# aymenboudhina/Multimodal_VQVAE_compression_audio_tactile

Hardware: AMD Instinct MI355X
Metric: encode+VQ+decode token-frames/sec (1 frame = 13.33 ms of paired 24 kHz audio+tactile) (higher is better)
Workload: dtype f32

## Files before the change

### multimodal_vqvae_compression_audio_tactile_amd/csrc/conv1d_mfma.hpp

```cpp
#pragma once
#include <hip/hip_runtime.h>
#include <stdio.h>
#include <stdlib.h>
#include <type_traits>
#include "det_math.hpp"
#include "kernels_small.hpp"

namespace mvq {

struct ConvArgs;
inline bool conv_dma_rows_ok(const ConvArgs& a);

__device__ __attribute__((aligned(16))) static const float g_zero16[4] = {0.0f, 0.0f, 0.0f, 0.0f};

int prof_begin(const char* kernel_name, double flops, hipStream_t s);
void prof_end(int idx, hipStream_t s);
bool prof_enabled();

typedef float f32x16 __attribute__((ext_vector_type(16)));
typedef float f32x4 __attribute__((ext_vector_type(4)));

struct ConvArgs {
    const float* x;
    const float* wp;
// ... 212 lines not shown
            __builtin_amdgcn_sched_barrier(0);
            run_from<S + 1>(acc, av0, bv0, av1, bv1, a_addr, b_same, b_cross);
        }
    }
};

constexpr int cgcd(int a, int b) { return b == 0 ? a : cgcd(b, a % b); }

template <int KS, int STRIDE, int DIL, int CK, int MT, int NT, int WAVES_M, int WAVES_N, int UPS>
struct ConvCfg {
    static constexpr int BM = 32 * MT * WAVES_M;
    static constexpr int BN = 32 * NT * WAVES_N;
    static constexpr int KC = CK * KS;
    static constexpr int XT = (BN - 1) * STRIDE + (KS - 1) * DIL + 1;
    static constexpr bool XALIGNED = (KS == 1 && STRIDE == 1);
    static constexpr int XV = XALIGNED ? (XT + 3) / 4 : (XT + 3 + 3) / 4;
    static constexpr int XTP = XV * 4 + 4;
    static constexpr int W_FLOATS = KC * BM;
    static constexpr int X_FLOATS = CK * XTP;
    static constexpr int STAGE_FLOATS = 2 * (W_FLOATS + X_FLOATS);
    static constexpr int BNP = BN + 4;
    static constexpr int CT_FLOATS = BM * BNP;
    static constexpr int EH = ((UPS == 0 || 32 % (UPS ? UPS : 1) == 0) && MT % 2 == 0 && CT_FLOATS > STAGE_FLOATS) ? 2 : 1;
    static constexpr int CTH_FLOATS = CT_FLOATS / EH;
    static constexpr int QPR = BN / 4;
    static constexpr int CQ = cgcd(QPR, 64 * WAVES_M * WAVES_N);
    static constexpr int JN = QPR / CQ;
    static constexpr int RSTEP = (64 * WAVES_M * WAVES_N) / CQ;
    static constexpr bool REG_GEOM = (UPS == 0) && (32 % RSTEP == 0);
    static constexpr int TB_FLOATS = REG_GEOM ? 2 * BM : 0;
    static constexpr int EPI_FLOATS = CTH_FLOATS + TB_FLOATS;
    static constexpr int EPI_FLOATS_FUSE = CT_FLOATS + TB_FLOATS;
    static constexpr int LDS_FLOATS = STAGE_FLOATS > EPI_FLOATS ? STAGE_FLOATS : EPI_FLOATS;
    static constexpr bool FOUR_WAVES = WAVES_M * WAVES_N == 4;
    static constexpr bool RING_FITS = (size_t)3 * (KC * BM + CK * XV * 4) * 4 <= 64 * 1024;
    static constexpr int MIN_WPE = (FOUR_WAVES && LDS_FLOATS * 4 <= 53 * 1024 && !(WAVES_N == 4 && NT == 2) && RING_FITS && MT * NT <= 4) ? 3
                                                                                                                : (WAVES_M * WAVES_N) / 2;
    static constexpr int LDS_FLOATS_FUSE = STAGE_FLOATS > EPI_FLOATS_FUSE ? STAGE_FLOATS : EPI_FLOATS_FUSE;
    static constexpr int MIN_WPE_FUSE = (FOUR_WAVES && (LDS_FLOATS_FUSE + 5 * BM) * 4 * 3 <= 160 * 1024) ? 3 : (WAVES_M * WAVES_N) / 2;
    static constexpr int XV4 = XV * 4;
    static constexpr int DMA_STAGE_FLOATS = W_FLOATS + CK * XV4;
    static constexpr int DMA_NV = DMA_STAGE_FLOATS / 4;
    static constexpr int DMA_NU = (DMA_NV + 64 * WAVES_M * WAVES_N - 1) / (64 * WAVES_M * WAVES_N);
    static constexpr int LDS_FLOATS_DMA = 3 * DMA_STAGE_FLOATS > EPI_FLOATS ? 3 * DMA_STAGE_FLOATS : EPI_FLOATS;
    static constexpr int LDS_FLOATS_FUSE_DMA = 3 * DMA_STAGE_FLOATS > EPI_FLOATS_FUSE ? 3 * DMA_STAGE_FLOATS : EPI_FLOATS_FUSE;
    static constexpr int W_VEC = W_FLOATS / 4;
    static constexpr int NTHR = 64 * WAVES_M * WAVES_N;
    static constexpr int W_PER_THREAD = (W_VEC + NTHR - 1) / NTHR;
    static constexpr int XV_TOTAL = CK * XV;
    static constexpr int XV_PER_THREAD = (XV_TOTAL + NTHR - 1) / NTHR;
    static constexpr int XS_TOTAL = CK * XT;
    static constexpr int XS_PER_THREAD = (XS_TOTAL + NTHR - 1) / NTHR;
    static constexpr int XREGS = (4 * XV_PER_THREAD > XS_PER_THREAD) ? 4 * XV_PER_THREAD : XS_PER_THREAD;
    static_assert(WAVES_M * WAVES_N == 4 || WAVES_M * WAVES_N == 8, "block is 4 or 8 waves");
    static_assert(KC % 2 == 0, "chunk K must be even (32x32x2 MFMA)");
    static_assert(BM % 4 == 0, "float4 weight staging");
};

template <int KS, int STRIDE, int DIL, int CK, int MT, int NT, int WAVES_M, int WAVES_N, int UPS, bool VEC>
struct ConvTile {
    using C = ConvCfg<KS, STRIDE, DIL, CK, MT, NT, WAVES_M, WAVES_N, UPS>;
    const float* wp; const float* xb; const float* Al;
    float* Ws; float* Xs;
    int tid, Tin, Cin, Mpad, m0, t_in0, g_al;
    bool snake_in;

    __device__ __forceinline__ void load_chunk(int chunk, f32x4 (&wreg)[C::W_PER_THREAD], f32x4 (&xv)[C::XV_PER_THREAD], float (&xs)[C::XS_PER_THREAD]) const
    {
        const int ci0 = chunk * CK;
        const float* wsrc = wp + (size_t)ci0 * KS * Mpad + m0;
#pragma unroll
        for (int u = 0; u < C::W_PER_THREAD; ++u) {
            int v = tid + u * C::NTHR;
            if (C::W_VEC % C::NTHR != 0) v = v < C::W_VEC ? v : C::W_VEC - 1;
            const int row = v / (C::BM / 4);
            const int c4 = v - row * (C::BM / 4);
            wreg[u] = *reinterpret_cast<const f32x4*>(wsrc + (size_t)row * Mpad + c4 * 4);
        }
        if (VEC) {
#pragma unroll
            for (int u = 0; u < C::XV_PER_THREAD; ++u) {
                int e = tid + u * C::NTHR;
                if (C::XV_TOTAL % C::NTHR != 0) e = e < C::XV_TOTAL ? e : C::XV_TOTAL - 1;
                const int cl = e / C::XV;
                const int v = e - cl * C::XV;
                const int g = g_al + 4 * v;
                const bool ok = g >= 0 && g < Tin;
                const int gc = ok ? g : 0;
                xv[u] = *reinterpret_cast<const f32x4*>(xb + (size_t)(ci0 + cl) * Tin + gc);
            }
        } else {
#pragma unroll
            for (int u = 0; u < C::XS_PER_THREAD; ++u) {
                int e = tid + u * C::NTHR;
                if (C::XS_TOTAL % C::NTHR != 0) e = e < C::XS_TOTAL ? e : C::XS_TOTAL - 1;
                const int cl = e / C::XT;
                const int xi = e - cl * C::XT;
                const int g = t_in0 + xi;
                const bool ok = g >= 0 && g < Tin;
                const int gc = ok ? g : 0;
                xs[u] = xb[(size_t)(ci0 + cl) * Tin + gc];
            }
        }
    }

    __device__ __forceinline__ void store_chunk(int chunk, int buf, const f32x4 (&wreg)[C::W_PER_THREAD],
                                                const f32x4 (&xv)[C::XV_PER_THREAD],
                                                const float (&xs)[C::XS_PER_THREAD]) const
    {
        const int ci0 = chunk * CK;
        float* wdst = Ws + buf * C::W_FLOATS;
        float* xdst = Xs + buf * C::X_FLOATS;
#pragma unroll
        for (int u = 0; u < C::W_PER_THREAD; ++u) {
            const int v = tid + u * C::NTHR;
            if (C::W_VEC % C::NTHR == 0 || v < C::W_VEC) *reinterpret_cast<f32x4*>(wdst + v * 4) = wreg[u];
        }
        if (VEC) {
#pragma unroll
            for (int u = 0; u < C::XV_PER_THREAD; ++u) {
                const int e = tid + u * C::NTHR;
                const int ec = (C::XV_TOTAL % C::NTHR != 0 && e >= C::XV_TOTAL) ? C::XV_TOTAL - 1 : e;
                const int cl = ec / C::XV;
                const int v = ec - cl * C::XV;
                const int g = g_al + 4 * v;
                const bool ok = g >= 0 && g < Tin;
                f32x4 q = xv[u];
                if (!ok) q = f32x4{0.0f, 0.0f, 0.0f, 0.0f};
                if (snake_in) {
                    const float al = Al[ci0 + cl], inv = Al[Cin + ci0 + cl];
                    q.x = det_snake(q.x, al, inv); q.y = det_snake(q.y, al, inv);
                    q.z = det_snake(q.z, al, inv); q.w = det_snake(q.w, al, inv);
                }
                if (C::XV_TOTAL % C::NTHR == 0 || e < C::XV_TOTAL)
                    *reinterpret_cast<f32x4*>(xdst + cl * C::XTP + 4 * v) = q;
            }
        } else {
#pragma unroll
            for (int u = 0; u < C::XS_PER_THREAD; ++u) {
                const int e = tid + u * C::NTHR;
                const int ec = (C::XS_TOTAL % C::NTHR != 0 && e >= C::XS_TOTAL) ? C::XS_TOTAL - 1 : e;
                const int cl = ec / C::XT;
                const int xi = ec - cl * C::XT;
                const int g = t_in0 + xi;
                float q = (g >= 0 && g < Tin) ? xs[u] : 0.0f;
                if (snake_in) q = det_snake(q, Al[ci0 + cl], Al[Cin + ci0 + cl]);
                if (C::XS_TOTAL % C::NTHR == 0 || e < C::XS_TOTAL) xdst[cl * C::XTP + xi] = q;
            }
        }
    }
};

template <int KS, int STRIDE, int DIL, int CK, int MT, int NT, int WAVES_M, int WAVES_N, int UPS, bool VEC, bool FUSE>
__device__ __forceinline__ void conv1d_mfma_body(const ConvArgs& a)
{
    using C = ConvCfg<KS, STRIDE, DIL, CK, MT, NT, WAVES_M, WAVES_N, UPS>;
    extern __shared__ __attribute__((aligned(16))) float smem[];
    float* const Ws = smem;
    float* const Xs = smem + 2 * C::W_FLOATS;
    float* const Ep = smem + (FUSE ? (a.dma ? C::LDS_FLOATS_FUSE_DMA : C::LDS_FLOATS_FUSE) : (a.dma ? C::LDS_FLOATS_DMA : C::LDS_FLOATS));
    constexpr int EP_MID = 2;
    float* const Al = Ep + 3 * C::BM;

    const int tid = threadIdx.x;
    const int lane = tid & 63;
    const int wave = tid >> 6;
    const int wm = wave / WAVES_N;
    const int wn = wave % WAVES_N;
    const int l31 = lane & 31;
    const int h = lane >> 5;

    int bx = blockIdx.x, by = blockIdx.y;
    if (a.row_fast) {
        const int xcd = bx & 7, j = bx >> 3;
        by = j % a.row_fast;
        bx = (j / a.row_fast) * 8 + xcd;
        if (bx >= a.n_tiles * a.B) return;
    }
    const int b = bx / a.n_tiles;
    const int tile_n = bx - b * a.n_tiles;
    const int n0 = a.n_base + tile_n * C::BN;
    const int m0 = by * C::BM;
    const int t_in0 = n0 * STRIDE - a.pad;
    const int g_al = t_in0 & ~3;
    const int shift = VEC ? (t_in0 - g_al) : 0;
    const int Cin = a.Cin;
    const int n_chunks = Cin / CK;
    const bool snake_in = a.alpha_in != nullptr;

    if (snake_in) {
        for (int c = tid; c < Cin; c += C::NTHR) {
            const float al = a.alpha_in[c];
            Al[c] = al;
            Al[Cin + c] = 1.0f / (al + 1e-9f);
        }
    }
    for (int r = tid; r < C::BM; r += C::NTHR) {
        int m = m0 + r;
        m = m < a.Mrows ? m : a.Mrows - 1;
        const int ch = m / (UPS ? UPS : 1);
        const float* tabs[4] = {a.alpha_out, a.y2 ? a.alpha2 : nullptr, FUSE ? a.alpha_mid : (a.dsn_src ? a.dsn_alpha : nullptr), nullptr};
#pragma unroll
        for (int k = 0; k < 3; ++k) {
            Ep[k * C::BM + r] = tabs[k] ? 1.0f / (tabs[k][ch] + 1e-9f) : 1.0f;
        }
    }

    ConvTile<KS, STRIDE, DIL, CK, MT, NT, WAVES_M, WAVES_N, UPS, VEC> tile;
    tile.wp = a.wp; tile.xb = a.x + (size_t)b * Cin * a.Tin; tile.Al = Al; tile.Ws = Ws; tile.Xs = Xs;
    tile.tid = tid; tile.Tin = a.Tin; tile.Cin = Cin; tile.Mpad = a.Mpad; tile.m0 = m0; tile.t_in0 = t_in0;
    tile.g_al = g_al; tile.snake_in = snake_in;

    f32x16 acc[MT][NT];
#pragma unroll
    for (int i = 0; i < MT; ++i)
#pragma unroll
        for (int j = 0; j < NT; ++j)
#pragma unroll
            for (int r = 0; r < 16; ++r) acc[i][j][r] = 0.0f;

    f32x4 wreg[C::W_PER_THREAD];
    f32x4 xv[C::XV_PER_THREAD];
    float xs[C::XS_PER_THREAD];

    constexpr int D_SAME = DIL;
    constexpr int D_CROSS = C::XTP - (KS - 1) * DIL;
    const int a_base = h * C::BM + wm * (MT * 32) + l31;
    const int b_base = (wn * (NT * 32) + l31) * STRIDE + shift;
    const int b_same = b_base + h * D_SAME;
    const int b_cross = b_base + h * D_CROSS;

    constexpr int NS = C::KC / 2;
    auto mfma_chunk = [&](int buf) __attribute__((always_inline)) {
        const float* wsrc = Ws + buf * C::W_FLOATS + a_base;
        const float* xs_same = Xs + buf * C::X_FLOATS + b_same;
        const float* xs_cross = Xs + buf * C::X_FLOATS + b_cross;
        float av[2][MT], bv[2][NT];
        auto load_step = [&](int st, int pb) __attribute__((always_inline)) {
            const int k0 = 2 * st;
            const int off0 = (k0 / KS) * C::XTP + (k0 % KS) * DIL;
            const bool cross = ((k0 + 1) / KS) != (k0 / KS);
            const float* xsp = cross ? xs_cross : xs_same;
#pragma unroll
            for (int i = 0; i < MT; ++i) av[pb][i] = wsrc[k0 * C::BM + i * 32];
#pragma unroll
            for (int j = 0; j < NT; ++j) bv[pb][j] = xsp[off0 + j * 32 * STRIDE];
        };
        load_step(0, 0);
#pragma unroll
        for (int s = 0; s < NS; ++s) {
            const int pb = s & 1;
            if (s + 1 < NS) load_step(s + 1, (s + 1) & 1);
#pragma unroll
            for (int i = 0; i < MT; ++i)
#pragma unroll
                for (int j = 0; j < NT; ++j)
                    acc[i][j] = __builtin_amdgcn_mfma_f32_32x32x2f32(av[pb][i], bv[pb][j], acc[i][j], 0, 0, 0);
            __builtin_amdgcn_sched_group_barrier(0x100, MT + NT, 0);
            __builtin_amdgcn_sched_group_barrier(0x008, MT * NT, 0);
        }
    };

    constexpr bool DMA_FITS = FUSE ? ((size_t)C::LDS_FLOATS_FUSE_DMA + 3 * C::BM) * 4 * 2 <= 160 * 1024 : (size_t)C::LDS_FLOATS_DMA * 4 <= 64 * 1024;
    bool use_dma = false;
    if constexpr (VEC && DMA_FITS) use_dma = a.dma != 0;
    if (use_dma) {
      if constexpr (VEC && DMA_FITS) {
        constexpr int NU = C::DMA_NU;
        constexpr int XP = C::XV4;
        constexpr int D_CROSS_D = XP - (KS - 1) * DIL;
        const int bd_same = b_base + h * D_SAME;
        const int bd_cross = b_base + h * D_CROSS_D;
        const unsigned lds0 = (unsigned)(size_t)smem;
        const int wave_u = __builtin_amdgcn_readfirstlane(wave);
        using AL = AsmOperandLoop<KS, STRIDE, DIL, C::BM, XP, MT, NT, NS>;
        auto chunk_rt = [&](int stage, auto&& issue) __attribute__((always_inline)) {
            const unsigned sb = lds0 + (unsigned)(stage * C::DMA_STAGE_FLOATS * 4);
            const unsigned a_addr = sb + (unsigned)(a_base * 4);
            const unsigned b_s = sb + (unsigned)((C::W_FLOATS + bd_same) * 4), b_c = sb + (unsigned)((C::W_FLOATS + bd_cross) * 4);
            float av0[MT], bv0[NT], av1[MT], bv1[NT];
            AL::template load_step<0>(av0, bv0, a_addr, b_s, b_c);
            issue();
            AL::template run_from<0>(acc, av0, bv0, av1, bv1, a_addr, b_s, b_c);
        };
        constexpr int NW = WAVES_M * WAVES_N;
        constexpr int XPC = CK * C::XV;
        constexpr int WI_W = (C::W_VEC + 63) / 64, WI_X = (XPC + 63) / 64;
        constexpr int NU_W = (WI_W + NW - 1) / NW, NU_X = (WI_X + NW - 1) / NW;
        constexpr int NF_W = C::W_VEC / C::NTHR, NF_X = XPC / C::NTHR;
        static_assert(NU_W - NF_W <= 1 && NU_X - NF_X <= 1, "at most one masked instruction per kind");
        constexpr int NI_MIN = (WI_W + WI_X) / NW;
        constexpr bool UNI_OK = (size_t)3 * C::DMA_STAGE_FLOATS * 4 <= 65536 && NF_W <= 8 && NF_X <= 8;
        bool uni = false;
        if constexpr (UNI_OK) uni = !a.vp_seg && g_al >= 0 && g_al + 4 * C::XV <= a.Tin && (long long)CK * a.Tin < (1ll << 29);
        if (uni) {
          if constexpr (UNI_OK) {
            unsigned woff[NU_W], xoff[NU_X];
#pragma unroll
            for (int u = 0; u < NU_W; ++u) {
                int p = tid + u * C::NTHR;
                p = p < C::W_VEC ? p : C::W_VEC - 1;
                const int row = p / (C::BM / 4), c4 = p - row * (C::BM / 4);
                woff[u] = (unsigned)(row * a.Mpad + c4 * 4) * 4u;
            }
            const int xw = (wave_u + NW - WI_W % NW) % NW;
#pragma unroll
            for (int j = 0; j < NU_X; ++j) {
                int q = (xw + j * NW) * 64 + lane;
                q = q < XPC ? q : XPC - 1;
                const int cl = q / C::XV, v = q - cl * C::XV;
                xoff[j] = (unsigned)(cl * a.Tin + 4 * v) * 4u;
            }
            unsigned long long mask_w = 0, mask_x = 0;
            if constexpr (NU_W > NF_W) mask_w = __ballot(tid + NF_W * C::NTHR < C::W_VEC);
            if constexpr (NU_X > NF_X) mask_x = __ballot((xw + NF_X * NW) * 64 + lane < XPC);
            unsigned long long wbase = dma_scalar_base(a.wp + m0);
            unsigned long long xbase = dma_scalar_base(tile.xb + g_al);
            const unsigned wstep = (unsigned)(CK * KS * a.Mpad) * 4u, xstep = (unsigned)(CK * a.Tin) * 4u;
            const unsigned wdst0 = lds0 + (unsigned)(wave_u * 1024), xdst0 = lds0 + (unsigned)(C::W_FLOATS * 4) + (unsigned)(xw * 1024);
            auto dma_uni = [&](int stage) __attribute__((always_inline)) {
                const unsigned so = (unsigned)(stage * C::DMA_STAGE_FLOATS * 4);
                if constexpr (NF_W > 0) lds_dma_burst_uni<NF_W, C::NTHR * 16>(woff, wbase, wdst0 + so);
                if constexpr (NU_W > NF_W) lds_dma_masked_uni(woff[NU_W - 1], wbase, wdst0 + so + (unsigned)(NF_W * C::NTHR * 16), mask_w);
                if constexpr (NF_X > 0) lds_dma_burst_uni<NF_X, C::NTHR * 16>(xoff, xbase, xdst0 + so);
                if constexpr (NU_X > NF_X) lds_dma_masked_uni(xoff[NU_X - 1], xbase, xdst0 + so + (unsigned)(NF_X * C::NTHR * 16), mask_x);
// ... 426 lines not shown
                else if (has_res && !hy2 && !snake_out) reg_quads(std::integral_constant<int, 5>{});
                else if (!has_res && !hy2 && !snake_out) reg_quads(std::integral_constant<int, 6>{});
                else reg_quads(std::integral_constant<int, 0>{});
            }
            if (quads_done) {
            } else if (PRE_RES) {
#pragma unroll
                for (int it = 0; it < RES_IT; ++it) quad(tid + it * C::NTHR, it);
            } else {
#pragma unroll 4
                for (int e = tid; e < NV; e += C::NTHR) quad(e, 0);
            }
        } else {
            constexpr int NE = BMH * C::BN;
#pragma unroll 4
            for (int e = tid; e < NE; e += C::NTHR) {
                const int row = e / C::BN;
                const int col = e - row * C::BN;
                const int m = m0 + tile_row(row), n = n0 + col;
                if (m < a.Mrows && n < a.Ncols) {
                    const size_t off = ((size_t)b * a.Cout + m) * a.Tout + n;
                    float v = Ct[row * C::BNP + col] + (ep_bias ? ep_bias[m] : 0.0f);
                    const int lr = tile_row(row);
                    if (a.dsn_src) v = v * det_dsnake(a.dsn_src[off], a.dsn_alpha[m], Ep[2 * C::BM + lr]);
                    if (has_res) v = v + a.residual[off];
                    bool tail = a.tvalid && n >= a.tvalid;
                    if (a.tper) tail = n - (int)__umulhi((unsigned)n, a.tper_magic) * a.tper >= a.tper_valid;
                    if (a.y2) a.y2[off] = tail ? 0.0f : det_snake(v, a.alpha2[m], Ep[C::BM + lr]);
                    if (snake_out) v = det_snake(v, a.alpha_out[m], Ep[lr]);
                    if (do_tanh) v = det_tanh(v);
                    if (do_gelu) v = det_gelu(v);
                    a.y[off] = tail ? 0.0f : v;
                }
            }
        }
    } else {
        constexpr int S = UPS ? UPS : 1;
        const int run = C::BN * S;
        const int nco = BMH / S;
        const int t_base = n0 * S - a.up_p;
        const int total = nco * run;
        auto shuffle_one = [&](int col, int tl) __attribute__((always_inline)) {
            const int nl = tl / S, rr = tl - nl * S;
            const int co = (m0 + tile_row(col * S)) / S;
            int t = t_base + tl;
            bool ok = co < a.Cout && n0 + nl < a.Ncols && t >= 0 && (a.up_per_out ? true : t < a.Tout);
            int bb = b;
            if (ok && a.up_per_out) {
                const int sg = (int)__umulhi((unsigned)t, a.up_magic);
                t -= sg * a.up_per_out;
                bb = b * a.up_seg + sg;
                ok = t < a.up_valid_out && bb < a.up_btrue;
            }
            if (ok) {
                float v = Ct[(col * S + rr) * C::BNP + nl] + (ep_bias ? ep_bias[co] : 0.0f);
                const size_t off = ((size_t)bb * a.Cout + co) * a.Tout + t;
                const bool tail = a.tvalid && t >= a.tvalid;
                const int lr = tile_row(col * S);
                if (a.y2) a.y2[off] = tail ? 0.0f : det_snake(v, a.alpha2[co], Ep[C::BM + lr]);
                if (snake_out) v = det_snake(v, a.alpha_out[co], Ep[lr]);
                a.y[off] = tail ? 0.0f : v;
            }
        };
        const bool up_quads = a.ovec4 && (C::BN * S) % 4 == 0 && (a.up_per_out == 0 || (a.up_per_out % 4 == 0 && a.up_valid_out % 4 == 0));
        if (up_quads) {
            const int lead = (4 - (t_base & 3)) & 3;
            const int QF = (run - lead) / 4;
            const int totq = nco * QF;
            for (int e = tid; e < totq; e += C::NTHR) {
                const int col = e / QF;
                const int tl0 = lead + 4 * (e - col * QF);
                const int co = (m0 + tile_row(col * S)) / S;
                int t = t_base + tl0;
                const int nl_last = (tl0 + 3) / S;
                bool ok = co < a.Cout && n0 + nl_last < a.Ncols && t >= 0 && (a.up_per_out ? true : t + 3 < a.Tout);
                int bb = b;
                if (ok && a.up_per_out) {
                    const int sg = (int)__umulhi((unsigned)t, a.up_magic);
                    t -= sg * a.up_per_out;
                    bb = b * a.up_seg + sg;
                    ok = t < a.up_valid_out && bb < a.up_btrue;
                } else if (!ok && co < a.Cout) {
#pragma unroll
                    for (int i = 0; i < 4; ++i) shuffle_one(col, tl0 + i);
                    continue;
                }
                if (!ok) continue;
                const float bv = ep_bias ? ep_bias[co] : 0.0f;
                f32x4 v;
#pragma unroll
                for (int i = 0; i < 4; ++i) {
                    const int tl = tl0 + i, nl = tl / S, rr = tl - nl * S;
                    v[i] = Ct[(col * S + rr) * C::BNP + nl] + bv;
                }
                const size_t off = ((size_t)bb * a.Cout + co) * a.Tout + t;
                const int lr = tile_row(col * S);
                int nz = (a.tvalid && t + 4 > a.tvalid) ? t + 4 - a.tvalid : 0;
                nz = nz > 4 ? 4 : nz;
                if (a.y2) {
                    const float a2 = a.alpha2[co], i2 = Ep[C::BM + lr];
                    f32x4 w = {det_snake(v.x, a2, i2), det_snake(v.y, a2, i2), det_snake(v.z, a2, i2), det_snake(v.w, a2, i2)};
                    if (nz > 0) { w.w = 0.0f; if (nz > 1) w.z = 0.0f; if (nz > 2) w.y = 0.0f; if (nz > 3) w.x = 0.0f; }
                    *reinterpret_cast<f32x4*>(a.y2 + off) = w;
                }
                if (snake_out) {
                    const float al = a.alpha_out[co], inv = Ep[lr];
                    v.x = det_snake(v.x, al, inv); v.y = det_snake(v.y, al, inv); v.z = det_snake(v.z, al, inv); v.w = det_snake(v.w, al, inv);
                }
                if (nz > 0) { v.w = 0.0f; if (nz > 1) v.z = 0.0f; if (nz > 2) v.y = 0.0f; if (nz > 3) v.x = 0.0f; }
                *reinterpret_cast<f32x4*>(a.y + off) = v;
            }
            const int rest = run - 4 * QF;
            for (int e = tid; e < nco * rest; e += C::NTHR) {
                const int col = e / rest, r = e - col * rest;
                shuffle_one(col, r < lead ? r : 4 * QF + r);
            }
        } else
        for (int e = tid; e < total; e += C::NTHR) {
            const int col = e / run;
            const int tl = e - col * run;
            const int nl = tl / S, rr = tl - nl * S;
            const int co = (m0 + tile_row(col * S)) / S;
            int t = t_base + tl;
            bool ok = co < a.Cout && n0 + nl < a.Ncols && t >= 0 && (a.up_per_out ? true : t < a.Tout);
            int bb = b;
            if (ok && a.up_per_out) {
                const int sg = (int)__umulhi((unsigned)t, a.up_magic);
                t -= sg * a.up_per_out;
                bb = b * a.up_seg + sg;
                ok = t < a.up_valid_out && bb < a.up_btrue;
            }
            if (ok) {
                float v = Ct[(col * S + rr) * C::BNP + nl] + (ep_bias ? ep_bias[co] : 0.0f);
                const size_t off = ((size_t)bb * a.Cout + co) * a.Tout + t;
                const bool tail = a.tvalid && t >= a.tvalid;
                const int lr = tile_row(col * S);
                if (a.y2) a.y2[off] = tail ? 0.0f : det_snake(v, a.alpha2[co], Ep[C::BM + lr]);
                if (snake_out) v = det_snake(v, a.alpha_out[co], Ep[lr]);
                a.y[off] = tail ? 0.0f : v;
            }
        }
    }
    };
    epilogue_pass(std::integral_constant<int, 0>{});
    if constexpr (EHP == 2) epilogue_pass(std::integral_constant<int, 1>{});
    static_assert(EHP == 1 || EHP == 2, "one or two epilogue passes");
}

template <int KS, int STRIDE, int DIL, int CK, int MT, int NT, int WAVES_M, int WAVES_N, int UPS>
__global__ __attribute__((amdgpu_flat_work_group_size(1, 64 * WAVES_M * WAVES_N),
                          amdgpu_waves_per_eu(ConvCfg<KS, STRIDE, DIL, CK, MT, NT, WAVES_M, WAVES_N, UPS>::MIN_WPE)))
void conv1d_mfma_kernel(const ConvArgs a)
{
    if (a.vec4) conv1d_mfma_body<KS, STRIDE, DIL, CK, MT, NT, WAVES_M, WAVES_N, UPS, true, false>(a);
    else conv1d_mfma_body<KS, STRIDE, DIL, CK, MT, NT, WAVES_M, WAVES_N, UPS, false, false>(a);
}

template <int DIL, int CK, int MT, int NT, int WAVES_M, int WAVES_N>
__global__ __attribute__((amdgpu_flat_work_group_size(1, 64 * WAVES_M * WAVES_N),
                          amdgpu_waves_per_eu(ConvCfg<7, 1, DIL, CK, MT, NT, WAVES_M, WAVES_N, 0>::MIN_WPE_FUSE)))
void residual_unit_kernel(const ConvArgs a)
{
    if (a.vec4) conv1d_mfma_body<7, 1, DIL, CK, MT, NT, WAVES_M, WAVES_N, 0, true, true>(a);
    else conv1d_mfma_body<7, 1, DIL, CK, MT, NT, WAVES_M, WAVES_N, 0, false, true>(a);
}

template <int DIL, int CK, int MT, int NT, int WAVES_M, int WAVES_N>
inline hipError_t launch_residual_unit(const ConvArgs& a_in, hipStream_t stream)
{
    using C = ConvCfg<7, 1, DIL, CK, MT, NT, WAVES_M, WAVES_N, 0>;
    ConvArgs a = a_in;
    if (a.Cin % CK != 0 || a.Cout != C::BM || a.Cin != C::BM || a.Mpad != C::BM) return hipErrorInvalidValue;
    if (a.name_out) {
        snprintf(a.name_out, a.name_len, "residual_unit_kernel<%d, %d, %d, %d, %d, %d>", DIL, CK, MT, NT, WAVES_M, WAVES_N);
        return hipSuccess;
    }
    a.n_tiles = (a.Ncols + C::BN - 1) / C::BN;
    a.vec4 = (a.Tin % 4 == 0) && ((reinterpret_cast<uintptr_t>(a.x) & 15) == 0);
    a.ovec4 = (a.Tout % 4 == 0) && ((reinterpret_cast<uintptr_t>(a.y) & 15) == 0) &&
              ((reinterpret_cast<uintptr_t>(a.residual) & 15) == 0);
    a.dma = (conv_dma_rows_ok(a) && ((size_t)C::LDS_FLOATS_FUSE_DMA + 3 * C::BM) * 4 * 2 <= 160 * 1024) ? 1 : 0;
    const size_t lds = a.dma ? (size_t)C::LDS_FLOATS_FUSE_DMA * 4 + (size_t)3 * C::BM * 4
                             : (size_t)C::LDS_FLOATS_FUSE * 4 + (size_t)3 * C::BM * 4 + (size_t)2 * a.Cin * 4;
    auto kern = residual_unit_kernel<DIL, CK, MT, NT, WAVES_M, WAVES_N>;
    {
        static BigLdsOptIn opt;
        const hipError_t e = opt.ensure(reinterpret_cast<const void*>(kern));
        if (e != hipSuccess) return e;
    }
    dim3 grid((unsigned)(a.n_tiles * a.B), 1);
    int pi = -1;
    if (prof_enabled()) {
        char nm[96];
        snprintf(nm, sizeof(nm), "residual_unit_kernel<%d, %d, %d, %d, %d, %d>", DIL, CK, MT, NT, WAVES_M, WAVES_N);
        const int cols = a.tvalid > 0 ? a.tvalid : a.Ncols;
        pi = prof_begin(nm, 2.0 * a.Cin * a.Cout * 8.0 * cols * a.B, stream);
    }
    hipLaunchKernelGGL(kern, grid, dim3(C::NTHR), lds, stream, a);
    prof_end(pi, stream);
    return hipGetLastError();
}

template <int KS, int STRIDE, int DIL, int CK, int MT, int NT, int WAVES_M, int WAVES_N, int UPS>
inline hipError_t launch_conv1d_mfma(const ConvArgs& a_in, hipStream_t stream)
{
    using C = ConvCfg<KS, STRIDE, DIL, CK, MT, NT, WAVES_M, WAVES_N, UPS>;
    ConvArgs a = a_in;
    if (a.Cin % CK != 0 || a.Mpad % C::BM != 0) return hipErrorInvalidValue;
    if (C::XALIGNED && (a.pad != 0 || a.n_base % 4 != 0)) return hipErrorInvalidValue;
    if (a.name_out) {
        snprintf(a.name_out, a.name_len, "conv1d_mfma_kernel<%d, %d, %d, %d, %d, %d, %d, %d, %d>", KS, STRIDE, DIL, CK, MT, NT,
                 WAVES_M, WAVES_N, UPS);
        return hipSuccess;
    }
    a.n_tiles = (a.Ncols - a.n_base + C::BN - 1) / C::BN;
    if (a.n_tiles_max > 0 && a.n_tiles > a.n_tiles_max) a.n_tiles = a.n_tiles_max;
    a.vec4 = (a.Tin % 4 == 0) && ((reinterpret_cast<uintptr_t>(a.x) & 15) == 0);
    a.ovec4 = (a.Tout % 4 == 0) && ((reinterpret_cast<uintptr_t>(a.y) & 15) == 0) &&
              (!a.residual || (reinterpret_cast<uintptr_t>(a.residual) & 15) == 0) &&
              (!a.y2 || (reinterpret_cast<uintptr_t>(a.y2) & 15) == 0) &&
              (!a.dsn_src || (reinterpret_cast<uintptr_t>(a.dsn_src) & 15) == 0);
    a.dma = (conv_dma_rows_ok(a) && (size_t)C::LDS_FLOATS_DMA * 4 <= 64 * 1024) ? 1 : 0;
    const size_t lds = (a.dma ? (size_t)C::LDS_FLOATS_DMA * 4 : (size_t)C::LDS_FLOATS * 4 + (a.alpha_in ? (size_t)2 * a.Cin * 4 : 0)) + (size_t)3 * C::BM * 4;
    auto kern = conv1d_mfma_kernel<KS, STRIDE, DIL, CK, MT, NT, WAVES_M, WAVES_N, UPS>;
    {
        static BigLdsOptIn opt;
        const hipError_t e = opt.ensure(reinterpret_cast<const void*>(kern));
        if (e != hipSuccess) return e;
    }
    if (lds > 160 * 1024) return hipErrorInvalidValue;
    if (a.vp_seg) {
        constexpr int EHP_ = C::EH, NVQ_ = (C::BM / EHP_) * C::BN / 4;
        constexpr bool REG_ = C::REG_GEOM && (NVQ_ % C::NTHR == 0) && (NVQ_ / C::NTHR <= 16) && ((C::BM / EHP_) % C::RSTEP == 0);
        if (!REG_ || UPS != 0 || !a.dma || !a.ovec4 || (a.y2 && a.alpha_out)) return hipErrorInvalidValue;
    }
    const unsigned gx = (unsigned)(a.n_tiles * a.B), R = (unsigned)((a.Mrows + C::BM - 1) / C::BM);
    dim3 grid(gx, R);
    a.row_fast = 0;
    if (R > 1 && (size_t)a.Cin * KS * a.Mpad * sizeof(float) <= ((size_t)5 << 19)) {
        a.row_fast = (int)R;
        grid = dim3(((gx + 7) / 8) * 8 * R, 1);
    }
    int pi = -1;
    if (prof_enabled()) {
        char nm[96];
        snprintf(nm, sizeof(nm), "conv1d_mfma_kernel<%d, %d, %d, %d, %d, %d, %d, %d, %d>", KS, STRIDE, DIL, CK, MT, NT, WAVES_M, WAVES_N, UPS);
        int last = a.n_base + a.n_tiles * C::BN;
        int lim = a.Ncols;
        if (UPS > 0 && !a.up_per_out) lim = a.Ncols - 1;
        else if (a.tvalid > 0) lim = a.tvalid;
        if (last > lim) last = lim;
        double cols = last > a.n_base ? last - a.n_base : 0;
        if (a.tper) cols *= (double)a.tper_valid / a.tper;
        if (a.vp_seg) cols *= ((double)a.vp_valid_out / a.vp_per_out) * ((double)a.vp_btrue / ((double)a.B * a.vp_seg));
        if (a.up_per_out) cols *= (double)a.up_valid_out / a.up_per_out;
        pi = prof_begin(nm, 2.0 * a.Cin * KS * a.Mrows * cols * a.B, stream);
    }
    hipLaunchKernelGGL(kern, grid, dim3(C::NTHR), lds, stream, a);
    prof_end(pi, stream);
    return hipGetLastError();
}

inline bool conv_dma_rows_ok(const ConvArgs& a)
{
    static const bool off = getenv("MVQ_NO_DMA") != nullptr;
    return !off && !a.alpha_in && a.Tin % 4 == 0 && (reinterpret_cast<uintptr_t>(a.x) & 15) == 0;
}

inline int conv_tile_bm(int mrows)
{
    if (mrows % 128 == 0) return 128;
    if (mrows % 96 == 0) return 96;
    if (mrows % 64 == 0) return 64;
    return mrows > 96 ? 128 : (mrows > 64 ? 96 : 64);
}
inline int conv_mpad(int mrows) { const int bm = conv_tile_bm(mrows); return (mrows + bm - 1) / bm * bm; }

inline int conv_tail_width(const ConvArgs& a)
{
    if (a.n_base != 0 || a.n_tiles_max != 0) return 0;
    if ((long)a.B * ((a.Mrows + 127) / 128) < 128) return 0;
    const int full = a.Ncols / 128, rem = a.Ncols % 128;
    if (full == 0 || rem == 0 || rem > 96) return 0;
    const int w = rem <= 64 ? 64 : 96;
    return (128 - w) * 100 >= (full + 1) * 128 ? w : 0;
}

inline bool conv_underfilled(const ConvArgs& a)
{
    return (long)a.B * ((a.Ncols + 127) / 128) * ((a.Mrows + 127) / 128) < 160;
}
inline bool conv_prefer_small_tiles(const ConvArgs& a)
{
    if (a.Mpad % 64 != 0) return false;
    if (a.vp_seg) return false;
    const long big = (long)a.B * ((a.Ncols + 127) / 128) * ((a.Mrows + 127) / 128);
    if (big < 160) return true;
    if (big >= 600) return false;
    const long small = 4 * big;
    const double fill_big = (double)big / (double)((big + 255) / 256 * 256);
    const double fill_small = (double)small / (double)((small + 255) / 256 * 256);
    return 0.85 * fill_small > fill_big;
}

}
```

### multimodal_vqvae_compression_audio_tactile_amd/csrc/conv_strided.hip

```cpp
#include "conv_dispatch.hpp"
namespace mvq {
hipError_t launch_conv_strided(const ConvArgs& a, int stride, int bm, hipStream_t s)
{
    const bool dma = conv_dma_rows_ok(a);
    if (bm == 96 && stride == 2) return dma ? launch_conv1d_mfma<4, 2, 1, 4, 3, 1, 1, 4, 0>(a, s) : launch_conv1d_mfma<4, 2, 1, 8, 3, 1, 1, 4, 0>(a, s);
    if (bm != 128) return hipErrorInvalidValue;
    if (conv_prefer_small_tiles(a)) {
        switch (stride) {
            case 2: return launch_conv1d_mfma<4, 2, 1, 16, 1, 1, 2, 2, 0>(a, s);
            case 4: return launch_conv1d_mfma<8, 4, 1, 8, 1, 1, 2, 2, 0>(a, s);
            case 5: return launch_conv1d_mfma<10, 5, 1, 4, 1, 1, 2, 2, 0>(a, s);
            case 8: return launch_conv1d_mfma<16, 8, 1, 4, 1, 1, 2, 2, 0>(a, s);
        }
    }
    const int tail = a.name_out ? 0 : conv_tail_width(a);
    if (tail && (stride == 4 || stride == 5)) {
        ConvArgs m = a, t = a;
        m.n_tiles_max = a.Ncols / 128;
        t.n_base = m.n_tiles_max * 128;
        hipError_t e = stride == 4 ? (dma ? launch_conv1d_mfma<8, 4, 1, 2, 2, 2, 2, 2, 0>(m, s) : launch_conv1d_mfma<8, 4, 1, 4, 2, 2, 2, 2, 0>(m, s))
                                   : launch_conv1d_mfma<10, 5, 1, 2, 2, 2, 2, 2, 0>(m, s);
        if (e != hipSuccess) return e;
        if (stride == 4) return tail == 96 ? launch_conv1d_mfma<8, 4, 1, 2, 1, 3, 4, 1, 0>(t, s) : launch_conv1d_mfma<8, 4, 1, 2, 2, 1, 2, 2, 0>(t, s);
        return tail == 96 ? launch_conv1d_mfma<10, 5, 1, 2, 1, 3, 4, 1, 0>(t, s) : launch_conv1d_mfma<10, 5, 1, 2, 2, 1, 2, 2, 0>(t, s);
    }
    switch (stride) {
        case 2: return dma ? launch_conv1d_mfma<4, 2, 1, 4, 2, 2, 2, 2, 0>(a, s) : launch_conv1d_mfma<4, 2, 1, 8, 2, 2, 2, 2, 0>(a, s);
        case 4: return dma ? launch_conv1d_mfma<8, 4, 1, 2, 2, 2, 2, 2, 0>(a, s) : launch_conv1d_mfma<8, 4, 1, 4, 2, 2, 2, 2, 0>(a, s);
        case 5: return launch_conv1d_mfma<10, 5, 1, 2, 2, 2, 2, 2, 0>(a, s);
        case 8: if (a.Ncols <= 96) return dma ? launch_conv1d_mfma<16, 8, 1, 1, 1, 3, 4, 1, 0>(a, s) : launch_conv1d_mfma<16, 8, 1, 2, 1, 3, 4, 1, 0>(a, s);
                return dma ? launch_conv1d_mfma<16, 8, 1, 1, 2, 2, 2, 2, 0>(a, s) : launch_conv1d_mfma<16, 8, 1, 2, 2, 2, 2, 2, 0>(a, s);
    }
    return hipErrorInvalidValue;
}
}
```

### multimodal_vqvae_compression_audio_tactile_amd/csrc/conv_tr.hip

```cpp
#include "conv_dispatch.hpp"
namespace mvq {
hipError_t launch_conv_tr(const ConvArgs& a, int bm, hipStream_t s)
{
    if (bm == 128 && conv_prefer_small_tiles(a)) {
        switch (a.up_s) {
            case 8: return launch_conv1d_mfma<2, 1, 1, 32, 1, 1, 2, 2, 8>(a, s);
            case 5: return launch_conv1d_mfma<2, 1, 1, 32, 1, 1, 2, 2, 5>(a, s);
            case 4: return launch_conv1d_mfma<2, 1, 1, 32, 1, 1, 2, 2, 4>(a, s);
            case 2: return launch_conv1d_mfma<2, 1, 1, 32, 1, 1, 2, 2, 2>(a, s);
        }
    }
    const bool dma = conv_dma_rows_ok(a);
    const int tail = (a.name_out || bm != 128) ? 0 : conv_tail_width(a);
    if (tail && (a.up_s == 4 || a.up_s == 5)) {
        ConvArgs m = a, t = a;
        m.n_tiles_max = a.Ncols / 128;
        t.n_base = m.n_tiles_max * 128;
        hipError_t e;
        if (a.up_s == 4) e = dma ? launch_conv1d_mfma<2, 1, 1, 8, 2, 2, 2, 2, 4>(m, s) : launch_conv1d_mfma<2, 1, 1, 16, 2, 2, 2, 2, 4>(m, s);
        else e = dma ? launch_conv1d_mfma<2, 1, 1, 8, 2, 2, 2, 2, 5>(m, s) : launch_conv1d_mfma<2, 1, 1, 16, 2, 2, 2, 2, 5>(m, s);
        if (e != hipSuccess) return e;
        if (a.up_s == 4) return tail == 96 ? launch_conv1d_mfma<2, 1, 1, 8, 1, 3, 4, 1, 4>(t, s) : launch_conv1d_mfma<2, 1, 1, 8, 2, 1, 2, 2, 4>(t, s);
        return tail == 96 ? launch_conv1d_mfma<2, 1, 1, 8, 1, 3, 4, 1, 5>(t, s) : launch_conv1d_mfma<2, 1, 1, 8, 2, 1, 2, 2, 5>(t, s);
    }
    const bool narrow = bm == 128 && a.Ncols <= 96;
    switch (a.up_s) {
        case 8: if (bm == 128 && narrow) return dma ? launch_conv1d_mfma<2, 1, 1, 8, 1, 3, 4, 1, 8>(a, s) : launch_conv1d_mfma<2, 1, 1, 16, 1, 3, 4, 1, 8>(a, s);
                if (bm == 128) return dma ? launch_conv1d_mfma<2, 1, 1, 8, 2, 2, 2, 2, 8>(a, s) : launch_conv1d_mfma<2, 1, 1, 16, 2, 2, 2, 2, 8>(a, s);
                break;
        case 5: if (bm == 128) return dma ? launch_conv1d_mfma<2, 1, 1, 8, 2, 2, 2, 2, 5>(a, s) : launch_conv1d_mfma<2, 1, 1, 16, 2, 2, 2, 2, 5>(a, s);
                break;
        case 4: if (bm == 128) return dma ? launch_conv1d_mfma<2, 1, 1, 8, 2, 2, 2, 2, 4>(a, s) : launch_conv1d_mfma<2, 1, 1, 16, 2, 2, 2, 2, 4>(a, s);
                break;
        case 2: if (bm == 96) return dma ? launch_conv1d_mfma<2, 1, 1, 8, 3, 1, 1, 4, 2>(a, s) : launch_conv1d_mfma<2, 1, 1, 16, 3, 1, 1, 4, 2>(a, s);
                if (bm == 128) return dma ? launch_conv1d_mfma<2, 1, 1, 8, 2, 2, 2, 2, 2>(a, s) : launch_conv1d_mfma<2, 1, 1, 16, 2, 2, 2, 2, 2>(a, s);
                break;
    }
    return hipErrorInvalidValue;
}
}
```

Baseline: 60400.

## Merge main and tail conv tile launches into one multi-range kernel

Adds a ranges kernel that runs the 128-column main tiles and the narrower tail tiles of a strided or transposed conv in a single launch. Each block works out from its index which range and tile configuration it belongs to. Launch planning is split into a reusable conv_plan helper. The goal is to cut a kernel launch and the serialization gap between the main and tail kernels, at the cost of a larger instantiated kernel whose register and occupancy bounds are set by the stricter of the two configurations.

```diff
diff --git a/multimodal_vqvae_compression_audio_tactile_amd/csrc/conv1d_mfma.hpp b/multimodal_vqvae_compression_audio_tactile_amd/csrc/conv1d_mfma.hpp
--- a/multimodal_vqvae_compression_audio_tactile_amd/csrc/conv1d_mfma.hpp
+++ b/multimodal_vqvae_compression_audio_tactile_amd/csrc/conv1d_mfma.hpp
@@ -388,7 +388,7 @@
 };
 
 template <int KS, int STRIDE, int DIL, int CK, int MT, int NT, int WAVES_M, int WAVES_N, int UPS, bool VEC, bool FUSE>
-__device__ __forceinline__ void conv1d_mfma_body(const ConvArgs& a)
+__device__ __forceinline__ void conv1d_mfma_body(const ConvArgs& a, const int bx_in, const int by_in)
 {
     using C = ConvCfg<KS, STRIDE, DIL, CK, MT, NT, WAVES_M, WAVES_N, UPS>;
     extern __shared__ __attribute__((aligned(16))) float smem[];
@@ -406,7 +406,7 @@
     const int l31 = lane & 31;
     const int h = lane >> 5;
 
-    int bx = blockIdx.x, by = blockIdx.y;
+    int bx = bx_in, by = by_in;
     if (a.row_fast) {
         const int xcd = bx & 7, j = bx >> 3;
         by = j % a.row_fast;
@@ -1139,8 +1139,8 @@
                           amdgpu_waves_per_eu(ConvCfg<KS, STRIDE, DIL, CK, MT, NT, WAVES_M, WAVES_N, UPS>::MIN_WPE)))
 void conv1d_mfma_kernel(const ConvArgs a)
 {
-    if (a.vec4) conv1d_mfma_body<KS, STRIDE, DIL, CK, MT, NT, WAVES_M, WAVES_N, UPS, true, false>(a);
-    else conv1d_mfma_body<KS, STRIDE, DIL, CK, MT, NT, WAVES_M, WAVES_N, UPS, false, false>(a);
+    if (a.vec4) conv1d_mfma_body<KS, STRIDE, DIL, CK, MT, NT, WAVES_M, WAVES_N, UPS, true, false>(a, (int)blockIdx.x, (int)blockIdx.y);
+    else conv1d_mfma_body<KS, STRIDE, DIL, CK, MT, NT, WAVES_M, WAVES_N, UPS, false, false>(a, (int)blockIdx.x, (int)blockIdx.y);
 }
 
 template <int DIL, int CK, int MT, int NT, int WAVES_M, int WAVES_N>
@@ -1148,8 +1148,8 @@
                           amdgpu_waves_per_eu(ConvCfg<7, 1, DIL, CK, MT, NT, WAVES_M, WAVES_N, 0>::MIN_WPE_FUSE)))
 void residual_unit_kernel(const ConvArgs a)
 {
-    if (a.vec4) conv1d_mfma_body<7, 1, DIL, CK, MT, NT, WAVES_M, WAVES_N, 0, true, true>(a);
-    else conv1d_mfma_body<7, 1, DIL, CK, MT, NT, WAVES_M, WAVES_N, 0, false, true>(a);
+    if (a.vec4) conv1d_mfma_body<7, 1, DIL, CK, MT, NT, WAVES_M, WAVES_N, 0, true, true>(a, (int)blockIdx.x, (int)blockIdx.y);
+    else conv1d_mfma_body<7, 1, DIL, CK, MT, NT, WAVES_M, WAVES_N, 0, false, true>(a, (int)blockIdx.x, (int)blockIdx.y);
 }
 
 template <int DIL, int CK, int MT, int NT, int WAVES_M, int WAVES_N>
@@ -1188,18 +1188,19 @@
     return hipGetLastError();
 }
 
+struct ConvPlan {
+    size_t lds;
+    unsigned gx, R;
+    unsigned blocks;
+    double flops;
+};
+
 template <int KS, int STRIDE, int DIL, int CK, int MT, int NT, int WAVES_M, int WAVES_N, int UPS>
-inline hipError_t launch_conv1d_mfma(const ConvArgs& a_in, hipStream_t stream)
+inline hipError_t conv_plan(ConvArgs& a, ConvPlan& p)
 {
     using C = ConvCfg<KS, STRIDE, DIL, CK, MT, NT, WAVES_M, WAVES_N, UPS>;
-    ConvArgs a = a_in;
     if (a.Cin % CK != 0 || a.Mpad % C::BM != 0) return hipErrorInvalidValue;
     if (C::XALIGNED && (a.pad != 0 || a.n_base % 4 != 0)) return hipErrorInvalidValue;
-    if (a.name_out) {
-        snprintf(a.name_out, a.name_len, "conv1d_mfma_kernel<%d, %d, %d, %d, %d, %d, %d, %d, %d>", KS, STRIDE, DIL, CK, MT, NT,
-                 WAVES_M, WAVES_N, UPS);
-        return hipSuccess;
-    }
     a.n_tiles = (a.Ncols - a.n_base + C::BN - 1) / C::BN;
     if (a.n_tiles_max > 0 && a.n_tiles > a.n_tiles_max) a.n_tiles = a.n_tiles_max;
     a.vec4 = (a.Tin % 4 == 0) && ((reinterpret_cast<uintptr_t>(a.x) & 15) == 0);
@@ -1208,51 +1209,157 @@
               (!a.y2 || (reinterpret_cast<uintptr_t>(a.y2) & 15) == 0) &&
               (!a.dsn_src || (reinterpret_cast<uintptr_t>(a.dsn_src) & 15) == 0);
     a.dma = (conv_dma_rows_ok(a) && (size_t)C::LDS_FLOATS_DMA * 4 <= 64 * 1024) ? 1 : 0;
-    const size_t lds = (a.dma ? (size_t)C::LDS_FLOATS_DMA * 4 : (size_t)C::LDS_FLOATS * 4 + (a.alpha_in ? (size_t)2 * a.Cin * 4 : 0)) + (size_t)3 * C::BM * 4;
+    p.lds = (a.dma ? (size_t)C::LDS_FLOATS_DMA * 4 : (size_t)C::LDS_FLOATS * 4 + (a.alpha_in ? (size_t)2 * a.Cin * 4 : 0)) + (size_t)3 * C::BM * 4;
+    if (p.lds > 160 * 1024) return hipErrorInvalidValue;
+    if (a.vp_seg) {
+        constexpr int EHP_ = C::EH, NVQ_ = (C::BM / EHP_) * C::BN / 4;
+        constexpr bool REG_ = C::REG_GEOM && (NVQ_ % C::NTHR == 0) && (NVQ_ / C::NTHR <= 16) && ((C::BM / EHP_) % C::RSTEP == 0);
+        if (!REG_ || UPS != 0 || !a.dma || !a.ovec4 || (a.y2 && a.alpha_out)) return hipErrorInvalidValue;
+    }
+    p.gx = (unsigned)(a.n_tiles * a.B);
+    p.R = (unsigned)((a.Mrows + C::BM - 1) / C::BM);
+    p.blocks = p.gx * p.R;
+    a.row_fast = 0;
+    if (p.R > 1 && (size_t)a.Cin * KS * a.Mpad * sizeof(float) <= ((size_t)5 << 19)) {
+        a.row_fast = (int)p.R;
+        p.blocks = ((p.gx + 7) / 8) * 8 * p.R;
+    }
+    int last = a.n_base + a.n_tiles * C::BN;
+    int lim = a.Ncols;
+    if (UPS > 0 && !a.up_per_out) lim = a.Ncols - 1;
+    else if (a.tvalid > 0) lim = a.tvalid;
+    if (last > lim) last = lim;
+    double cols = last > a.n_base ? last - a.n_base : 0;
+    if (a.tper) cols *= (double)a.tper_valid / a.tper;
+    if (a.vp_seg) cols *= ((double)a.vp_valid_out / a.vp_per_out) * ((double)a.vp_btrue / ((double)a.B * a.vp_seg));
+    if (a.up_per_out) cols *= (double)a.up_valid_out / a.up_per_out;
+    p.flops = 2.0 * a.Cin * KS * a.Mrows * cols * a.B;
+    return hipSuccess;
+}
+
+template <int KS, int STRIDE, int DIL, int CK, int MT, int NT, int WAVES_M, int WAVES_N, int UPS>
+inline hipError_t launch_conv1d_mfma(const ConvArgs& a_in, hipStream_t stream)
+{
+    using C = ConvCfg<KS, STRIDE, DIL, CK, MT, NT, WAVES_M, WAVES_N, UPS>;
+    ConvArgs a = a_in;
+    if (a.name_out) {
+        if (a.Cin % CK != 0 || a.Mpad % C::BM != 0) return hipErrorInvalidValue;
+        if (C::XALIGNED && (a.pad != 0 || a.n_base % 4 != 0)) return hipErrorInvalidValue;
+        snprintf(a.name_out, a.name_len, "conv1d_mfma_kernel<%d, %d, %d, %d, %d, %d, %d, %d, %d>", KS, STRIDE, DIL, CK, MT, NT,
+                 WAVES_M, WAVES_N, UPS);
+        return hipSuccess;
+    }
     auto kern = conv1d_mfma_kernel<KS, STRIDE, DIL, CK, MT, NT, WAVES_M, WAVES_N, UPS>;
     {
         static BigLdsOptIn opt;
         const hipError_t e = opt.ensure(reinterpret_cast<const void*>(kern));
         if (e != hipSuccess) return e;
     }
-    if (lds > 160 * 1024) return hipErrorInvalidValue;
-    if (a.vp_seg) {
-        constexpr int EHP_ = C::EH, NVQ_ = (C::BM / EHP_) * C::BN / 4;
-        constexpr bool REG_ = C::REG_GEOM && (NVQ_ % C::NTHR == 0) && (NVQ_ / C::NTHR <= 16) && ((C::BM / EHP_) % C::RSTEP == 0);
-        if (!REG_ || UPS != 0 || !a.dma || !a.ovec4 || (a.y2 && a.alpha_out)) return hipErrorInvalidValue;
-    }
-    const unsigned gx = (unsigned)(a.n_tiles * a.B), R = (unsigned)((a.Mrows + C::BM - 1) / C::BM);
-    dim3 grid(gx, R);
-    a.row_fast = 0;
-    if (R > 1 && (size_t)a.Cin * KS * a.Mpad * sizeof(float) <= ((size_t)5 << 19)) {
-        a.row_fast = (int)R;
-        grid = dim3(((gx + 7) / 8) * 8 * R, 1);
-    }
+    ConvPlan p;
+    const hipError_t pe = conv_plan<KS, STRIDE, DIL, CK, MT, NT, WAVES_M, WAVES_N, UPS>(a, p);
+    if (pe != hipSuccess) return pe;
+    const dim3 grid = a.row_fast ? dim3(p.blocks, 1) : dim3(p.gx, p.R);
     int pi = -1;
     if (prof_enabled()) {
         char nm[96];
         snprintf(nm, sizeof(nm), "conv1d_mfma_kernel<%d, %d, %d, %d, %d, %d, %d, %d, %d>", KS, STRIDE, DIL, CK, MT, NT, WAVES_M, WAVES_N, UPS);
-        int last = a.n_base + a.n_tiles * C::BN;
-        int lim = a.Ncols;
-        if (UPS > 0 && !a.up_per_out) lim = a.Ncols - 1;
-        else if (a.tvalid > 0) lim = a.tvalid;
-        if (last > lim) last = lim;
-        double cols = last > a.n_base ? last - a.n_base : 0;
-        if (a.tper) cols *= (double)a.tper_valid / a.tper;
-        if (a.vp_seg) cols *= ((double)a.vp_valid_out / a.vp_per_out) * ((double)a.vp_btrue / ((double)a.B * a.vp_seg));
-        if (a.up_per_out) cols *= (double)a.up_valid_out / a.up_per_out;
-        pi = prof_begin(nm, 2.0 * a.Cin * KS * a.Mrows * cols * a.B, stream);
-    }
-    hipLaunchKernelGGL(kern, grid, dim3(C::NTHR), lds, stream, a);
+        pi = prof_begin(nm, p.flops, stream);
+    }
+    hipLaunchKernelGGL(kern, grid, dim3(C::NTHR), p.lds, stream, a);
     prof_end(pi, stream);
     return hipGetLastError();
 }
 
+constexpr int CONV_MAX_RANGES = 2;
+struct ConvRangeArgs {
+    ConvArgs a[CONV_MAX_RANGES];
+    int nblk[CONV_MAX_RANGES];
+    int period;
+};
+template <int N>
+__device__ __forceinline__ int conv_range_of(const int (&nblk)[N], int& r)
+{
+    int k = 0;
+#pragma unroll
+    for (int i = 0; i + 1 < N; ++i)
+        if (k == i && r >= nblk[i]) { r -= nblk[i]; k = i + 1; }
+    return k;
+}
+
+constexpr int cmin(int a, int b) { return a < b ? a : b; }
+
+template <int KS, int STRIDE, int DIL, int CK, int UPS, int MT0, int NT0, int WM0, int WN0, int MT1, int NT1, int WM1, int WN1>
+__global__ __attribute__((amdgpu_flat_work_group_size(1, 256),
+                          amdgpu_waves_per_eu(cmin(ConvCfg<KS, STRIDE, DIL, CK, MT0, NT0, WM0, WN0, UPS>::MIN_WPE,
+                                                   ConvCfg<KS, STRIDE, DIL, CK, MT1, NT1, WM1, WN1, UPS>::MIN_WPE))))
+void conv1d_mfma_ranges_kernel(const ConvRangeArgs g)
+{
+    static_assert(WM0 * WN0 == 4 && WM1 * WN1 == 4, "every range is a four-wave block");
+    const int bid = blockIdx.x;
+    const int by = __builtin_amdgcn_readfirstlane(bid / g.period);
+    int r = __builtin_amdgcn_readfirstlane(bid - by * g.period);
+    const int k = conv_range_of(g.nblk, r);
+    if (k == 0) conv1d_mfma_body<KS, STRIDE, DIL, CK, MT0, NT0, WM0, WN0, UPS, true, false>(g.a[0], r, by);
+    else conv1d_mfma_body<KS, STRIDE, DIL, CK, MT1, NT1, WM1, WN1, UPS, true, false>(g.a[1], r, by);
+}
+
+template <int KS, int STRIDE, int DIL, int CK, int UPS, int MT0, int NT0, int WM0, int WN0, int MT1, int NT1, int WM1, int WN1>
+inline hipError_t launch_conv1d_mfma_ranges(const ConvArgs& a_in, hipStream_t stream)
+{
+    using C0 = ConvCfg<KS, STRIDE, DIL, CK, MT0, NT0, WM0, WN0, UPS>;
+    using C1 = ConvCfg<KS, STRIDE, DIL, CK, MT1, NT1, WM1, WN1, UPS>;
+    static_assert(C0::BN == 128 && C0::BM == C1::BM, "main range: 128-column tiles; both ranges share the row tiling");
+    static_assert((size_t)C0::LDS_FLOATS_DMA * 4 <= 64 * 1024 && (size_t)C1::LDS_FLOATS_DMA * 4 <= 64 * 1024, "both rings must fit");
+    if (a_in.name_out || a_in.n_base != 0 || a_in.n_tiles_max != 0 || a_in.Ncols < 128) return hipErrorInvalidValue;
+    ConvRangeArgs g;
+    g.a[0] = a_in;
+    g.a[1] = a_in;
+    g.a[0].n_tiles_max = a_in.Ncols / 128;
+    g.a[1].n_base = g.a[0].n_tiles_max * 128;
+    ConvPlan p[CONV_MAX_RANGES];
+    hipError_t e = conv_plan<KS, STRIDE, DIL, CK, MT0, NT0, WM0, WN0, UPS>(g.a[0], p[0]);
+    if (e != hipSuccess) return e;
+    e = conv_plan<KS, STRIDE, DIL, CK, MT1, NT1, WM1, WN1, UPS>(g.a[1], p[1]);
+    if (e != hipSuccess) return e;
+    if (!g.a[0].dma || !g.a[1].dma || p[0].R != p[1].R || g.a[0].row_fast != g.a[1].row_fast) return hipErrorInvalidValue;
+    unsigned nblocks;
+    if (g.a[0].row_fast) {
+        g.nblk[0] = (int)p[0].blocks;
+        g.nblk[1] = (int)p[1].blocks;
+        g.period = g.nblk[0] + g.nblk[1];
+        nblocks = (unsigned)g.period;
+    } else {
+        g.nblk[0] = (int)p[0].gx;
+        g.nblk[1] = (int)p[1].gx;
+        g.period = g.nblk[0] + g.nblk[1];
+        nblocks = (unsigned)g.period * p[0].R;
+    }
+    const size_t lds = p[0].lds > p[1].lds ? p[0].lds : p[1].lds;
+    auto kern = conv1d_mfma_ranges_kernel<KS, STRIDE, DIL, CK, UPS, MT0, NT0, WM0, WN0, MT1, NT1, WM1, WN1>;
+    {
+        static BigLdsOptIn opt;
+        e = opt.ensure(reinterpret_cast<const void*>(kern));
+        if (e != hipSuccess) return e;
+    }
+    int pi = -1;
+    if (prof_enabled()) {
+        char nm[128];
+        snprintf(nm, sizeof(nm), "conv1d_mfma_ranges_kernel<%d, %d, %d, %d, %d, %d, %d, %d, %d, %d, %d, %d, %d>", KS, STRIDE, DIL, CK, UPS,
+                 MT0, NT0, WM0, WN0, MT1, NT1, WM1, WN1);
+        pi = prof_begin(nm, p[0].flops + p[1].flops, stream);
+    }
+    hipLaunchKernelGGL(kern, dim3(nblocks), dim3(256), lds, stream, g);
+    prof_end(pi, stream);
+    return hipGetLastError();
+}
+
 inline bool conv_dma_rows_ok(const ConvArgs& a)
 {
     static const bool off = getenv("MVQ_NO_DMA") != nullptr;
     return !off && !a.alpha_in && a.Tin % 4 == 0 && (reinterpret_cast<uintptr_t>(a.x) & 15) == 0;
 }
+
+inline bool conv_ranges_ok(const ConvArgs& a) { return conv_dma_rows_ok(a) && !a.dsn_src; }
 
 inline int conv_tile_bm(int mrows)
 {
diff --git a/multimodal_vqvae_compression_audio_tactile_amd/csrc/conv_strided.hip b/multimodal_vqvae_compression_audio_tactile_amd/csrc/conv_strided.hip
--- a/multimodal_vqvae_compression_audio_tactile_amd/csrc/conv_strided.hip
+++ b/multimodal_vqvae_compression_audio_tactile_amd/csrc/conv_strided.hip
@@ -14,6 +14,12 @@
         }
     }
     const int tail = a.name_out ? 0 : conv_tail_width(a);
+    if (tail && stride == 4 && conv_ranges_ok(a))
+        return tail == 96 ? launch_conv1d_mfma_ranges<8, 4, 1, 2, 0, 2, 2, 2, 2, 1, 3, 4, 1>(a, s)
+                          : launch_conv1d_mfma_ranges<8, 4, 1, 2, 0, 2, 2, 2, 2, 2, 1, 2, 2>(a, s);
+    if (tail && stride == 5 && conv_ranges_ok(a))
+        return tail == 96 ? launch_conv1d_mfma_ranges<10, 5, 1, 2, 0, 2, 2, 2, 2, 1, 3, 4, 1>(a, s)
+                          : launch_conv1d_mfma_ranges<10, 5, 1, 2, 0, 2, 2, 2, 2, 2, 1, 2, 2>(a, s);
     if (tail && (stride == 4 || stride == 5)) {
         ConvArgs m = a, t = a;
         m.n_tiles_max = a.Ncols / 128;
diff --git a/multimodal_vqvae_compression_audio_tactile_amd/csrc/conv_tr.hip b/multimodal_vqvae_compression_audio_tactile_amd/csrc/conv_tr.hip
--- a/multimodal_vqvae_compression_audio_tactile_amd/csrc/conv_tr.hip
+++ b/multimodal_vqvae_compression_audio_tactile_amd/csrc/conv_tr.hip
@@ -12,6 +12,9 @@
     }
     const bool dma = conv_dma_rows_ok(a);
     const int tail = (a.name_out || bm != 128) ? 0 : conv_tail_width(a);
+    if (tail && dma && a.up_s == 4 && conv_ranges_ok(a))
+        return tail == 96 ? launch_conv1d_mfma_ranges<2, 1, 1, 8, 4, 2, 2, 2, 2, 1, 3, 4, 1>(a, s)
+                          : launch_conv1d_mfma_ranges<2, 1, 1, 8, 4, 2, 2, 2, 2, 2, 1, 2, 2>(a, s);
     if (tail && (a.up_s == 4 || a.up_s == 5)) {
         ConvArgs m = a, t = a;
         m.n_tiles_max = a.Ncols / 128;
```

Result: no change. 60290 (-0.2%).
